# regeirk/pycwt

Hardware: NVIDIA H100
Metric: cwt_scale_points_per_sec (higher is better)
Workload: dtype f64

## Files before the change

### profiles/micro/coarse_ab.py

```python
import os
import subprocess
import sys

import numpy as np

ROOT = os.path.dirname(os.path.dirname(os.path.dirname(os.path.abspath(__file__))))
sys.path.insert(0, ROOT)
import workloads as wl
import pycwt_b200 as pycwt
from pycwt_b200 import _engine
from pycwt_b200.wavelet import _boxcar_len
from bench import pin_to_gpu_numa_node


def identical(arms, fn):
    a, b = (fn(e) for e in arms.values())
    if isinstance(a, tuple):
        return all(np.array_equal(x, y) for x, y in zip(a, b) if x is not None)
    return np.array_equal(a, b)


def main():
    args = sys.argv[1:]
    parent = args[0]
    new = args[1] if len(args) > 1 and not args[1].isdigit() else os.path.join(ROOT, "pycwt_b200", "libcwtb200.so")
    rounds = int(args[-1]) if args[-1].isdigit() else 6
    pin_to_gpu_numa_node(0)
    print(subprocess.run(["nvidia-smi", "--query-gpu=name,power.limit,clocks.max.sm", "--format=csv"],
                         capture_output=True, text=True).stdout.strip())
    c = wl.C2
    x = wl.config2_signal()
    sj = wl.config2_scales()
    arms = {"parent": _engine.Engine(0, lib_path=parent), "new": _engine.Engine(0, lib_path=new)}
    dev = {}
    launches = {}
    for name, eng in arms.items():
        d = eng.dev_alloc(x.nbytes)
        eng.h2d(d, x)
        eng.cwt_dev(d, 0, c["n"], c["dt"], sj, _engine.MORLET, c["f0"], _engine.F64)
        eng.bench_last(10)
        launches[name] = eng.last_launch_count()
        dev[name] = d
    times = {k: [] for k in arms}
    for _ in range(rounds):
        for name, eng in arms.items():
            times[name].append(eng.bench_last(20))
    for name, t in times.items():
        print("%-6s config 2 step %.4f ms (min %.4f, max %.4f) over %d runs of 20 steps, %d launches per step" % (
            name, float(np.median(t)), min(t), max(t), len(t), launches[name]))
    print("median difference parent - new: %.4f ms" % (float(np.median(times["parent"])) - float(np.median(times["new"]))))
    for name, eng in arms.items():
        print(name + ": serialised kernels of one step")
        for k in sorted(eng.profile_last(), key=lambda k: -k["ms"]):
            print("      %-52s %3d x  %7.4f ms  rows %d" % (k["name"], k["launches"], k["ms"], k["rows"]))
    same = True
    for r0 in range(0, len(sj), 32):

        rows = []
        for eng in arms.values():
            out = np.empty((32, c["n"]), np.complex128)
            eng._check(eng.lib.cwtb_get_w(eng.h, _engine._ptr(out), 1, r0, 32))
            rows.append(out)
        same = same and np.array_equal(rows[0], rows[1])
    print("config 2 W (fp64, 256 rows): %s" % ("bit-identical" if same else "DIFFERENT"))
    for name, eng in arms.items():
        eng.dev_free(dev[name])
    c3 = wl.C3
    x3 = wl.config3_signal()
    for fam, code in (("dog", _engine.DOG), ("paul", _engine.PAUL)):
        p = c3[fam]
        s3 = wl.geometric_scales(p["s0"], p["dj"], p["J"])
        for name, eng in arms.items():
            d = eng.dev_alloc(x3.nbytes)
            eng.h2d(d, x3)
            eng.cwt_dev(d, 1, c3["n"], c3["dt"], s3, code, float(p["m"]), _engine.F32)
            eng.bench_last(10)
            launches[name] = eng.last_launch_count()
            dev[name] = d
        times = {k: [] for k in arms}
        for _ in range(rounds):
            for name, eng in arms.items():
                times[name].append(eng.bench_last(20))
        for name, t in times.items():
            print("%-6s config 3 %-4s step %.4f ms (min %.4f, max %.4f), %d launches per step" % (
                name, fam, float(np.median(t)), min(t), max(t), launches[name]))
        for name, eng in arms.items():
            print("%s: serialised kernels of one config 3 %s step" % (name, fam))
            for k in sorted(eng.profile_last(), key=lambda k: -k["ms"]):
                print("      %-52s %3d x  %7.4f ms  rows %d" % (k["name"], k["launches"], k["ms"], k["rows"]))
            eng.dev_free(dev[name])
    print("config 3 Paul(4) W (fp32): %s" % ("bit-identical" if identical(
        arms, lambda e: e.cwt(x3, c3["dt"], s3, _engine.PAUL, float(p["m"]), _engine.F32)) else "DIFFERENT"))
    c4 = wl.C4
    y1, y2 = wl.config4_signals()
    s4 = wl.geometric_scales(c4["s0"], c4["dj"], c4["J"])
    klen = _boxcar_len(pycwt.Morlet(c4["f0"]), c4["dj"])
    for prec, pname in ((_engine.F64, "fp64"), (_engine.F32, "fp32")):
        ok_x = identical(arms, lambda e: e.xwt(y1, y2, c4["dt"], s4, _engine.MORLET, c4["f0"], prec))
        ok_w = identical(arms, lambda e: e.wct(y1, y2, c4["dt"], c4["dj"], s4, _engine.MORLET, c4["f0"], klen,
                                               True, prec))
        print("config 4 %s: xwt %s, wct %s" % (pname, "bit-identical" if ok_x else "DIFFERENT",
                                               "bit-identical" if ok_w else "DIFFERENT"))
    for eng in arms.values():
        eng.close()


if __name__ == "__main__":
    main()
```

### pycwt_b200/csrc/engine.cu

```cuda
#include <algorithm>
#include <array>
#include <cmath>
#include <cstdint>
#include <cstdio>
#include <cstdlib>
#include <cstring>
#include <map>
#include <mutex>
#include <set>
#include <string>
#include <type_traits>
#include <vector>

#include <cuda_runtime.h>
#ifndef CWTB_HOST_EMU
#include <dlfcn.h>
#endif

#include "../../include/cwt_b200.h"
#include "kernels.cuh"

using namespace cwtb;

template <class B, class = void> struct BodyNT { static constexpr int value = NT; };
// ... 92 lines not shown
  int log2N = 0;
  int S = 0;
  int nbatch = 1;
  double dt = 0;
  Fam fam{};
  std::vector<ScaleDesc> descs;
  std::vector<ClassRun> classes;
  std::vector<int> plan_log2K;
  std::vector<double> scales;
  size_t b_single = 0;
  size_t coarse_elems = 0;
  int sig_is_f32 = 0;
  bool exact = false;
  std::vector<OsGroup> os_groups;
};

struct BluePlan {
  unsigned n = 0, L = 0;
  double2 *wm = nullptr;
  double2 *bf[2] = {nullptr, nullptr};
};

struct NTabDev {
  double2 *hi = nullptr, *lo = nullptr;
  int h = 0;
};

struct cwtb_ctx {
  int device = 0;
  rt_stream stream{};
  rt_stream aux_stream{};
  rt_stream prio_stream{};
  rt_stream prio_short{};
  int prio_mode = 1;
  rt_stream chain_streams[3]{};
  int n_chains = 2;
  rt_stream cur{};
  int pad_pow2 = 1;
  int coh_precision = 0;
  std::map<unsigned, BluePlan> blue;
  long long serial = 0;
  int two_streams = 1;
  int three_streams = 1;
  rt_stream copy_streams[4]{};
  int d2h_split = 1;
  std::string err;
  double band_eps = 1e-16;
  double band_eps32 = 1e-9;
  double expand_eps = 5e-13;
  double expand_eps32 = 2e-7;
  int expand_mma = 1;
  int dense_margin = 2;
  int expand_min_log2R = 0;
  int os_on = 1;
  Buf osH, osgrp;
  void *comm = nullptr;
  int comm_world = 1, comm_rank = 0;
  Buf comm_send, comm_recv;
  int group = 0;
  size_t group_bytes = (size_t)512 << 20;
  size_t rows_chunk_bytes = (size_t)256 << 20;
  int l2_persist = 0;
  int direct_max_log2 = 13;
  int fused = 0;
  int ring = 3;
  int pipe_ahead = 2;
  int num_sms = 132;
// ... 749 lines not shown
}

template <typename T> struct FusedArgs {
  PassAArgs<T> a;
  PassBArgs<T> b;
  unsigned *ctr;
  int nscales, ring;
  unsigned tilesA, tilesB;
};

HD void fused_decode(unsigned t, int n, unsigned TA, unsigned TB, int *isB, int *s, unsigned *tile) {
  if (t < TA) { *isB = 0; *s = 0; *tile = t; return; }
  t -= TA;
  const unsigned per = TA + TB;
  const unsigned blk = t / per, off = t % per;
  if ((int)blk < n - 1) {
    if (off < TA) { *isB = 0; *s = (int)blk + 1; *tile = off; }
    else { *isB = 1; *s = (int)blk; *tile = off - TA; }
  } else {
    *isB = 1; *s = n - 1; *tile = t - (unsigned)(n - 1) * per;
  }
}

#ifndef CWTB_HOST_EMU
__device__ __forceinline__ unsigned ld_acquire_u32(const unsigned *p) {
  unsigned v;
  asm volatile("ld.acquire.gpu.global.u32 %0, [%1];" : "=r"(v) : "l"(p) : "memory");
  return v;
}
template <typename T, int K1, int MODE>
__global__ void __launch_bounds__(TileCfg<T>::NT, 3) k_fused(const __grid_constant__ FusedArgs<T> f) {
  extern __shared__ __align__(16) unsigned char smraw[];
  __shared__ unsigned s_t;
  using A = PassABody<T, K1, MODE, +1>;
  using B = PassBBody<T, +1>;
  const int n = f.nscales;
  const unsigned total = (unsigned)n * (f.tilesA + f.tilesB);
  unsigned *doneA = f.ctr + 1, *doneB = f.ctr + 1 + n;
  for (;;) {
    __syncthreads();
    if (threadIdx.x == 0) s_t = atomicAdd(f.ctr, 1u);
    __syncthreads();
    const unsigned t = s_t;
    if (t >= total) break;
    int isB, s;
    unsigned tile;
    fused_decode(t, n, f.tilesA, f.tilesB, &isB, &s, &tile);
    if (threadIdx.x == 0) {
      if (isB) {
        while (ld_acquire_u32(&doneA[s]) < f.tilesA) __nanosleep(100);
      } else if (s >= f.ring) {
        while (ld_acquire_u32(&doneB[s - f.ring]) < f.tilesB) __nanosleep(100);
      }
      asm volatile("fence.proxy.async;" ::: "memory");
    }
    __syncthreads();
    if (isB) run_phases_at<B, 0>(f.b, (int)tile, s, smraw);
    else run_phases_at<A, 0>(f.a, (int)tile, s, smraw);
    __syncthreads();
    if (threadIdx.x == 0)
      asm volatile("red.release.gpu.global.add.u32 [%0], %1;" ::"l"(isB ? &doneB[s] : &doneA[s]), "r"(1u) : "memory");
  }
}
#endif

template <typename T, int K1, int MODE>
static int launch_fused(cwtb_ctx *c, const PassAArgs<T> &a, const PassBArgs<T> &b, int nscales) {
  using A = PassABody<T, K1, MODE, +1>;
  using B = PassBBody<T, +1>;
  FusedArgs<T> f;
  f.a = a; f.b = b;
  f.nscales = nscales;
  f.ring = c->ring;
  f.a.zmod = f.b.zmod = c->ring;
  const unsigned M = a.N / ((unsigned)K1 * K2C);
  f.tilesA = M * (K2C / A::T2);
  f.tilesB = (a.N / K2C + Lay<T, K2C>::P - 1) / Lay<T, K2C>::P;
  int e = ensure(c, c->ctr, (size_t)(1 + 2 * nscales) * sizeof(unsigned));
  if (e) return e;
  f.ctr = (unsigned *)c->ctr.p;
  RT(rt_memset(c->ctr.p, 0, (size_t)(1 + 2 * nscales) * sizeof(unsigned), c->stream));
#ifdef CWTB_HOST_EMU
  std::vector<unsigned char> sm(std::max(A::SMEM, B::SMEM) + 64);
  const unsigned total = (unsigned)nscales * (f.tilesA + f.tilesB);
  for (unsigned t = 0; t < total; ++t) {
    int isB, s;
    unsigned tile;
    fused_decode(t, nscales, f.tilesA, f.tilesB, &isB, &s, &tile);
    if (isB) emu_phases<B, 0>(f.b, (int)tile, s, sm.data());
    else emu_phases<A, 0>(f.a, (int)tile, s, sm.data());
  }
  c->launches++;
  return 0;
#else
  const size_t smem = std::max(A::SMEM, B::SMEM);
  auto kern = k_fused<T, K1, MODE>;
  const void *fn = (const void *)kern;
  if (!c->configured.count(fn)) {
    RT(cudaFuncSetAttribute(kern, cudaFuncAttributeMaxDynamicSharedMemorySize, (int)smem));
    c->configured.insert(fn);
  }
// ... 36 lines not shown
    case 10: return launch_fused<T, 1024, MODE>(c, a, b, n);
  }
  return fail(c, CWTB_ERR_UNSUPPORTED, "transform longer than 2^20 per row is not supported yet");
}

template <typename T> struct PipeArgs {
  PassAArgs<T> a;
  PassBArgs<T> b;
  unsigned *ctr;
  int nscales, ring, ahead;
  unsigned tilesA, tilesB;
};

HD void pipe_decode(unsigned t, int n, int ahead, unsigned TA, unsigned TB, int *isB, int *s, unsigned *tile) {
  const int na = ahead < n ? ahead : n;
  if (t < (unsigned)na * TA) { *isB = 0; *s = (int)(t / TA); *tile = t % TA; return; }
  t -= (unsigned)na * TA;
  const unsigned per = TA + TB;
  const int nmid = n - na;
  if (t < (unsigned)nmid * per) {
    const unsigned blk = t / per, off = t % per;
    if (off < TA) { *isB = 0; *s = na + (int)blk; *tile = off; }
    else { *isB = 1; *s = (int)blk; *tile = off - TA; }
    return;
  }
  t -= (unsigned)nmid * per;
  *isB = 1; *s = nmid + (int)(t / TB); *tile = t % TB;
}

#ifndef CWTB_HOST_EMU
template <typename T, int K1, int MODE>
__global__ void __launch_bounds__(TileCfg<T>::NT, 3) k_pipe(const __grid_constant__ PipeArgs<T> f) {
  extern __shared__ __align__(16) unsigned char smraw[];
  using A = PassABody<T, K1, MODE, +1>;
  using B = PassBBody<T, +1>;
  const int n = f.nscales;
  const unsigned total = (unsigned)n * (f.tilesA + f.tilesB);
  unsigned *doneA = f.ctr, *doneB = f.ctr + n;
  int okA = -1, okB = -1;
  for (unsigned t = blockIdx.x; t < total; t += gridDim.x) {
    int isB, s;
    unsigned tile;
    pipe_decode(t, n, f.ahead, f.tilesA, f.tilesB, &isB, &s, &tile);
    const int dep = isB ? s : s - f.ring;
    if (dep >= 0 && dep > (isB ? okA : okB)) {
      if (threadIdx.x == 0) {
        const unsigned *flag = isB ? &doneA[dep] : &doneB[dep];
        const unsigned want = isB ? f.tilesA : f.tilesB;
        while (ld_acquire_u32(flag) < want) __nanosleep(64);
        asm volatile("fence.proxy.async;" ::: "memory");
      }
      __syncthreads();
      if (isB) okA = dep; else okB = dep;
    }
    if (isB) run_phases_at<B, 0>(f.b, (int)tile, s, smraw);
    else run_phases_at<A, 0>(f.a, (int)tile, s, smraw);
    __syncthreads();
    if (threadIdx.x == blockDim.x - 1) {
      asm volatile("red.release.gpu.global.add.u32 [%0], %1;" ::"l"(isB ? &doneB[s] : &doneA[s]), "r"(1u) : "memory");
    }
  }
}
#endif

template <typename T, int K1, int MODE>
static int launch_pipe(cwtb_ctx *c, const PassAArgs<T> &a, const PassBArgs<T> &b, int nscales) {
  using A = PassABody<T, K1, MODE, +1>;
  using B = PassBBody<T, +1>;
  PipeArgs<T> f;
  f.a = a; f.b = b;
  f.nscales = nscales;
  f.ring = c->ring;
  f.ahead = std::max(1, std::min(c->pipe_ahead, c->ring - 1));
  f.a.zmod = f.b.zmod = c->ring;
  f.b.rev = 0; f.b.pf_dist = 0; f.a.pf_dist = 0;
  const unsigned M = a.N / ((unsigned)K1 * K2C);
  f.tilesA = M * (K2C / A::T2);
  f.tilesB = (a.N / K2C + Lay<T, K2C>::P - 1) / Lay<T, K2C>::P;
  int e = ensure(c, c->ctr, (size_t)(2 * nscales) * sizeof(unsigned));
  if (e) return e;
  f.ctr = (unsigned *)c->ctr.p;
  RT(rt_memset(c->ctr.p, 0, (size_t)(2 * nscales) * sizeof(unsigned), c->cur));
#ifdef CWTB_HOST_EMU
  std::vector<unsigned char> sm(std::max(A::SMEM, B::SMEM) + 64);
  const unsigned total = (unsigned)nscales * (f.tilesA + f.tilesB);
  std::vector<int> seenA(nscales, 0), seenB(nscales, 0);
  for (unsigned t = 0; t < total; ++t) {
    int isB, s;
    unsigned tile;
    pipe_decode(t, nscales, f.ahead, f.tilesA, f.tilesB, &isB, &s, &tile);
    if (isB && seenA[s] != (int)f.tilesA) return fail(c, CWTB_ERR_STATE, "pipe schedule: B before its A tiles");
    if (!isB && s >= f.ring && seenB[s - f.ring] != (int)f.tilesB)
      return fail(c, CWTB_ERR_STATE, "pipe schedule: Z slot reused before its B tiles");
    if (isB) { emu_phases<B, 0>(f.b, (int)tile, s, sm.data()); seenB[s]++; }
    else { emu_phases<A, 0>(f.a, (int)tile, s, sm.data()); seenA[s]++; }
  }
  c->launches++;
  return 0;
#else
  const size_t smem = std::max(A::SMEM, B::SMEM);
// ... 674 lines not shown
int cwtb_host_free(cwtb_ctx *c, void *p) {
  if (!c || !c->pinned.count(p)) return CWTB_ERR_ARG;
  c->pinned.erase(p);
  rt_host_free(p);
  return 0;
}
int cwtb_dev_alloc(cwtb_ctx *c, size_t bytes, void **out) {
  if (!c || !out) return CWTB_ERR_ARG;
  if (rt_malloc(out, bytes) != 0) return fail(c, CWTB_ERR_NOMEM, "device allocation failed");
  c->devallocs.insert(*out);
  return 0;
}
int cwtb_dev_free(cwtb_ctx *c, void *p) {
  if (!c || !c->devallocs.count(p)) return CWTB_ERR_ARG;
  c->devallocs.erase(p);
  rt_free(p);
  return 0;
}
int cwtb_memcpy_h2d(cwtb_ctx *c, void *dst, const void *src, size_t bytes) {
  RT(rt_h2d(dst, src, bytes, c->stream));
  RT(rt_sync(c->stream));
  return 0;
}
int cwtb_memcpy_d2h(cwtb_ctx *c, void *dst, const void *src, size_t bytes) {
  RT(rt_d2h(dst, src, bytes, c->stream));
  RT(rt_sync(c->stream));
  return 0;
}
int cwtb_sync(cwtb_ctx *c) {
  RT(rt_sync(c->stream));
  return 0;
}

static const double kOsUs = 9.5;
static const double kTwoKernelUs = 23.2;

struct DevTmp {
  void *p = nullptr;
  ~DevTmp() { if (p) rt_free(p); }
};

static int os_plan(cwtb_ctx *c, const Job &job, double dt, int family, double param, std::vector<OsRow> &os) {
  constexpr int L = OsBody<4>::L, GR = 4;
  auto os_cheaper = [](int M) { return M <= L / 2 && kOsUs * L / (double)(L - M + 1) < kTwoKernelUs; };
  os.assign(job.S, OsRow());
  const unsigned N = job.N;
  if (!c->os_on || job.precision != CWTB_F64 || job.exact || family == CWTB_TABLE ||
      !(c->band_eps > 0) || !(c->expand_eps > 0) || N < 2u * L)
    return 0;
  const long long half = (long long)N / 2;
  std::vector<int> cand;
  std::vector<double> cs;
  for (const ScaleDesc &d : job.descs) {
    if (d.chan != 0 || d.k_hi < d.k_lo || d.k_lo <= -half || d.k_hi >= ((long long)N - 1) / 2) continue;
    if (d.ip_log2Nc || (d.log2K <= 10 || (d.log2K <= c->direct_max_log2 && d.log2K < job.log2N))) continue;
    cand.push_back(d.row);
    cs.push_back(d.s);
  }
  if (cand.empty()) return 0;
  const int nc = (int)cand.size();
  const size_t wcap = (size_t)job.S * job.nbatch * job.n0;
  const int chunk = (int)std::max<size_t>(1, wcap / N);
  int e = ensure(c, c->W, std::max<size_t>((size_t)chunk * N, wcap) * sizeof(double2));
  if (e) return e;
  double2 *h = (double2 *)c->W.p;
  DevTmp dimp, part;
  if (rt_malloc(&dimp.p, (size_t)N * sizeof(double))) return fail(c, CWTB_ERR_NOMEM, "device allocation failed");
  {
// ... 1546 lines not shown
```

### pycwt_b200/csrc/fft_tile.cuh

```cuda
#pragma once
#include "cplx.cuh"

namespace cwtb {

#ifndef CWTB_NT
#define CWTB_NT 128
#endif
#ifndef CWTB_NT_F32
#define CWTB_NT_F32 256
#endif
#ifndef CWTB_TILE_F64
#define CWTB_TILE_F64 4096
#endif
#ifndef CWTB_TILE_F32
#define CWTB_TILE_F32 8192
#endif
#ifndef CWTB_MINB
#define CWTB_MINB 1
#endif
#ifndef CWTB_UNROLL_B
#define CWTB_UNROLL_B 1
#endif
#define CWTB_STR_(x) #x
#define CWTB_STR(x) CWTB_STR_(x)
#define CWTB_PRAGMA_UNROLL_B _Pragma(CWTB_STR(unroll CWTB_UNROLL_B))
#ifndef CWTB_PASSA_BATCH
#define CWTB_PASSA_BATCH 8
#endif
#ifndef CWTB_UNROLL_A
#define CWTB_UNROLL_A 4
#endif
#define CWTB_PRAGMA_UNROLL_A _Pragma(CWTB_STR(unroll CWTB_UNROLL_A))
constexpr int NT = CWTB_NT;
#ifndef CWTB_PLAN1024_R32
#define CWTB_PLAN1024_R32 0
#endif
#ifndef CWTB_PLAN256_3PASS
#define CWTB_PLAN256_3PASS 1
#endif
HD constexpr int tw_radix(int L) {
  return L == 32 ? 4 : (L == 256 ? (CWTB_PLAN256_3PASS ? 4 : 16) : ((L == 1024 && CWTB_PLAN1024_R32) ? 32 : 8));
}
// ... 210 lines not shown
    V e = nroot_t<T>(nt, (unsigned)base * pk2);
    const V se = nroot_t<T>(nt, (unsigned)stride * pk2);
    const V ne = nroot_t<T>(nt, (unsigned)(-K) * pk2);
#pragma unroll
    for (int i = 0; i < R; ++i) {
      tw[i] = (base + i * stride >= rsplit_row) ? cmul(e, ne) : e;
      e = cmul(e, se);
    }
  }
  HD void load(int b, V (&x)[R]) const {
#pragma unroll
    for (int i = 0; i < R; ++i) x[i] = cmul(sm[Lay<T, K>::phys(b, base + i * stride)], tw[i]);
  }
};

template <typename T, int K> struct RowLoader {
  using V = cx<T>;
  const V *src;
  int nvalid;
  int base, stride;
  HD void begin(int base_, int stride_, int, int) { base = base_; stride = stride_; }
  template <int R> HD void load(int b, V (&x)[R]) const {
    if (b < nvalid) {
      const V *row = src + (size_t)b * K + base;
#pragma unroll
      for (int i = 0; i < R; ++i) x[i] = row[i * stride];
    } else {
#pragma unroll
      for (int i = 0; i < R; ++i) x[i] = mk<T>(0, 0);
    }
  }
};

template <typename T, int K, int R> struct GenLoader {
  using V = cx<T>;
  static constexpr int P = Lay<T, K>::P;
  static constexpr int I = K / R;
  static constexpr int NT = TileCfg<T>::NT;
  static constexpr int GROUPS = (I >= NT) ? 1 : NT / I;
  static constexpr bool ONE_SHOT = (P / GROUPS <= 1);
  const V *B;
  NTab nt;
  int rsplit;
  unsigned p0;
  V a[ONE_SHOT ? 1 : R], d[ONE_SHOT ? 1 : R];
  int base, stride;
  unsigned pp;
  HD void begin(int base_, int stride_, int bstart, int bstep) {
    base = base_; stride = stride_;
    pp = p0 + (unsigned)bstart;
    if (ONE_SHOT) return;
    V e = nroot_t<T>(nt, (unsigned)base * pp);
    V de = nroot_t<T>(nt, (unsigned)base * (unsigned)bstep);
    const V se = nroot_t<T>(nt, (unsigned)stride * pp);
    const V sd = nroot_t<T>(nt, (unsigned)stride * (unsigned)bstep);
    const V ne = nroot_t<T>(nt, (unsigned)(-K) * pp);
    const V nd = nroot_t<T>(nt, (unsigned)(-K) * (unsigned)bstep);
#pragma unroll
    for (int i = 0; i < R; ++i) {
      const int r = base + i * stride;
      const bool neg = r >= rsplit;
      d[ONE_SHOT ? 0 : i] = neg ? cmul(de, nd) : de;
      a[ONE_SHOT ? 0 : i] = cmul(ldg(&B[r]), neg ? cmul(e, ne) : e);
      e = cmul(e, se);
      de = cmul(de, sd);
    }
  }
  HD void load(int, V (&x)[R]) {
    if (ONE_SHOT) {
      V e = nroot_t<T>(nt, (unsigned)base * pp);
      const V se = nroot_t<T>(nt, (unsigned)stride * pp);
      const V ne = nroot_t<T>(nt, (unsigned)(-K) * pp);
#pragma unroll
      for (int i = 0; i < R; ++i) {
        const int r = base + i * stride;
        x[i] = cmul(ldg(&B[r]), (r >= rsplit) ? cmul(e, ne) : e);
        e = cmul(e, se);
      }
      return;
    }
#pragma unroll
    for (int i = 0; i < R; ++i) { x[i] = a[ONE_SHOT ? 0 : i]; a[ONE_SHOT ? 0 : i] = cmul(a[ONE_SHOT ? 0 : i], d[ONE_SHOT ? 0 : i]); }
  }
};

template <typename T, int K, int L, int R, int SIGN, class Loader, bool ROWS = false>
HD void pass_mid(cx<T> *sm, const cx<T> *__restrict__ tw, Loader &ld, int tid) {
  using V = cx<T>;
  using LY = Lay<T, K, ROWS>;
  constexpr int NT = TileCfg<T>::NT;
  constexpr int Ln = L / R, I = K / R, P = LY::P;
  constexpr int LANES = (I >= NT) ? NT : I;
  constexpr int GROUPS = NT / LANES;
  const int tp0 = tid % LANES, bg = tid / LANES;
  for (int tp = tp0; tp < I; tp += LANES) {
    const int g = tp / Ln, j = tp % Ln;
    V twv[R];
#pragma unroll
    static_assert(tw_radix(L) == R, "pass twiddle table was built for another radix");
    for (int c = 1; c < R; ++c) {
      V w = ldg(&tw[tw_offset(L) + (c - 1) * Ln + j]);
      if (SIGN < 0) w.y = -w.y;
      twv[c] = w;
    }
    ld.begin(g * L + j, Ln, bg, GROUPS);
    CWTB_PRAGMA_UNROLL_B
    for (int b = bg; b < P; b += GROUPS) {
      V x[R];
      ld.load(b, x);
      dftR<R, SIGN, T>(x);
#pragma unroll
      for (int c = 1; c < R; ++c) x[c] = cmul(x[c], twv[c]);
#pragma unroll
      for (int c = 0; c < R; ++c) sm[LY::phys(b, g * L + c * Ln + j)] = x[c];
    }
  }
}

template <typename T, int K, int SIGN, class Storer, bool ROWS = false, bool GMAJOR = false>
HD void pass_last(const cx<T> *sm, Storer &st, int tid) {
  using V = cx<T>;
  using LY = Lay<T, K, ROWS>;
  constexpr int NT = TileCfg<T>::NT;
  constexpr int R = Plan<K>::RL, G = K / R, P = LY::P;
  for (int idx = tid; idx < G * P; idx += NT) {
    const int b = GMAJOR ? idx / G : idx % P, g = GMAJOR ? idx % G : idx / P;
    V x[R];
#pragma unroll
    for (int i = 0; i < R; ++i) x[i] = sm[LY::phys(b, g * R + i)];
    dftR<R, SIGN, T>(x);
    st.store(b, Plan<K>::qlow(g), G, x);
  }
}

template <typename T, int K> struct TilePhases {
  static constexpr int NP = Plan<K>::NP;
};

template <typename T, int K, int SIGN, class Loader, bool ROWS = false>
HD void tile_first(cx<T> *sm, const cx<T> *tw, Loader &ld, int tid) {
  pass_mid<T, K, K, Plan<K>::R1, SIGN, Loader, ROWS>(sm, tw, ld, tid);
}
template <typename T, int K, int SIGN, bool ROWS = false>
HD void tile_second(cx<T> *sm, const cx<T> *tw, int tid) {
  SmemLoader<T, K, ROWS> ld;
  ld.sm = sm;
  pass_mid<T, K, K / Plan<K>::R1, Plan<K>::R2, SIGN, SmemLoader<T, K, ROWS>, ROWS>(sm, tw, ld, tid);
}

}
```

### pycwt_b200/csrc/kernels.cuh

```cuda
#pragma once
#include <math.h>
#include "fft_tile.cuh"

namespace cwtb {

struct ScaleDesc {
  double s;
  double amp;
  int row;
  int k_lo, k_hi;
  int log2K;
  int rsplit;
  int trow;
  int chan;
  int pad_;
  long long boff;
  int ip_log2Nc;
  int ip_kc;
  int ip_w;
  int os_grp;
  long long ip_coff;
  long long ip_woff;
  double ip_beta;
  double ip_dc;
// ... 402 lines not shown
      st.U = U;
      st.ostride = il;
      st.ooff = (a.by0 + by) % il;
      st.epi.mode = a.epi;
      if (a.epi == EPI_GAUSS) {
        st.epi.g = a.grow[row];
        st.epi.invn = 1.0 / ((double)a.N * il);
        st.epi.post = a.post;
        st.epi.nfreq = (long long)a.N * il;
      }
      pass_last<T, K, SIGN, OutStorer<T>, true>(sm, st, tid);
      if (tid == 0) tb.inval();
    }
  }
};

struct OsGroup {
  int first, count;
  int t1, hop;
  long long hoff;
};
struct OsArgs {
  const ScaleDesc *descs;
  const OsGroup *groups;
  const double *sig;
  const double2 *H;
  double2 *W;
  const double2 *tw;
  long long n0;
  unsigned N;
  int epi;
};

template <int L, int R> struct OsSigLoader {
  const double *x;
  long long start, n0;
  unsigned nmask;
  int hop, base, stride;
  HD void begin(int base_, int stride_, int, int) { base = base_; stride = stride_; }
  HD void load(int b, double2 (&v)[R]) const {
    const long long s = start + (long long)b * hop + base;
#pragma unroll
    for (int i = 0; i < R; ++i) {
      const long long n = (s + (long long)i * stride) & (long long)nmask;
      v[i] = make_double2(n < n0 ? ldg(&x[n]) : 0.0, 0.0);
    }
  }
};
template <int L> struct OsHalfStorer {
  double2 *xs;
  template <int R> HD void store(int b, int ql, int qs, double2 (&x)[R]) const {
#pragma unroll
    for (int c = 0; c < R; ++c) {
      const int q = ql + c * qs;
      if (q <= L / 2) xs[b * (L / 2 + 1) + q] = x[c];
    }
  }
};
template <int L, int R> struct OsSpecLoader {
  const double2 *xs, *H;
  int base, stride;
  double2 hv[R];
  HD void begin(int base_, int stride_, int, int) {
    base = base_; stride = stride_;
#pragma unroll
    for (int i = 0; i < R; ++i) hv[i] = ldg(&H[base + i * stride]);
  }
  HD void load(int b, double2 (&v)[R]) const {
#pragma unroll
    for (int i = 0; i < R; ++i) {
      const int q = base + i * stride;
      const double2 y = q <= L / 2 ? xs[b * (L / 2 + 1) + q] : cconj(xs[b * (L / 2 + 1) + L - q]);
      v[i] = cmul(y, hv[i]);
    }
  }
};
struct OsStorer {
  double2 *row;
  long long nb0, n0;
  int t1, hop, epi;
  template <int R> HD void store(int b, int ql, int qs, double2 (&x)[R]) const {
    const long long nb = nb0 + (long long)b * hop;
#pragma unroll
    for (int c = 0; c < R; ++c) {
      const int i = ql + c * qs;
      const long long n = nb + i;
      if (i >= t1 && i < t1 + hop && n < n0) {
        if (epi == EPI_STORE) st_stream(&row[n], x[c]);
        else row[n] = cmul(row[n], cconj(x[c]));
      }
    }
  }
};

template <int G> struct OsBody {
  static constexpr int L = 1024;
  static constexpr int NTB = TileCfg<double>::NT;
  static constexpr int NT = NTB;
  using Args = OsArgs;
  using LY = Lay<double, L>;
  static constexpr int P = LY::P;
  static_assert(Plan<L>::NP == 3, "overlap-save phases assume a three-pass tile plan");
  static constexpr int NPHASE = 3 + 3 * G;
  static constexpr size_t SMEM = LY::TILE_BYTES + (size_t)P * (L / 2 + 1) * sizeof(double2);
  template <int PH> HD static void phase(const Args &a, int bx, int by, int tid, void *smraw) {
    double2 *sm = (double2 *)smraw;
    double2 *xs = (double2 *)((char *)smraw + LY::TILE_BYTES);
    const OsGroup g = a.groups[by];
    const long long n_first = (long long)bx * P * g.hop;
    if (n_first >= a.n0) return;
    if constexpr (PH == 0) {
      OsSigLoader<L, Plan<L>::R1> ld;
      ld.x = a.sig + (size_t)a.descs[g.first].chan * a.n0; ld.start = n_first - g.t1; ld.n0 = a.n0; ld.nmask = a.N - 1; ld.hop = g.hop;
      tile_first<double, L, -1>(sm, a.tw, ld, tid);
    } else if constexpr (PH == 1) {
      tile_second<double, L, -1>(sm, a.tw, tid);
    } else if constexpr (PH == 2) {
      OsHalfStorer<L> st{xs};
      pass_last<double, L, -1, OsHalfStorer<L>, false, true>(sm, st, tid);
    } else {
      constexpr int r = (PH - 3) / 3, step = (PH - 3) % 3;
      if (r >= g.count) return;
      if constexpr (step == 0) {
        OsSpecLoader<L, Plan<L>::R1> ld;
        ld.xs = xs; ld.H = a.H + g.hoff + (long long)r * L;
        tile_first<double, L, +1>(sm, a.tw, ld, tid);
      } else if constexpr (step == 1) {
        tile_second<double, L, +1>(sm, a.tw, tid);
      } else {
        OsStorer st;
        st.row = a.W + (size_t)a.descs[g.first + r].row * a.n0;
        st.nb0 = n_first - g.t1; st.n0 = a.n0; st.t1 = g.t1; st.hop = g.hop; st.epi = a.epi;
        pass_last<double, L, +1, OsStorer, false, true>(sm, st, tid);
      }
    }
  }
};

struct AbsMaxArgs { const double2 *h; double *out; long long pitch, lo, hi; int nblk; };
struct AbsMaxBody {
  using Args = AbsMaxArgs;
  static constexpr int NPHASE = 2;
  static constexpr size_t SMEM = NT * sizeof(double);
  template <int PH> HD static void phase(const Args &a, int bx, int by, int tid, void *smraw) {
    double *sm = (double *)smraw;
    if constexpr (PH == 0) {
      const long long chunk = (a.hi - a.lo + a.nblk - 1) / a.nblk;
      const long long s = a.lo + bx * chunk, e = s + chunk < a.hi ? s + chunk : a.hi;
      double m = 0;
      for (long long i = s + tid; i < e; i += NT) {
        const double2 v = a.h[(size_t)by * a.pitch + i];
        m = fmax(m, fmax(fabs(v.x), fabs(v.y)));
      }
      sm[tid] = m;
    } else if (tid == 0) {
      double m = 0;
      for (int i = 0; i < NT; ++i) m = fmax(m, sm[i]);
      a.out[(size_t)by * a.nblk + bx] = m;
    }
  }
};

enum { MODE_DENSE = 0, MODE_BAND = 1, MODE_REAL = 2, MODE_CPLX = 3, MODE_COARSE = 4 };

template <typename T> HD cx<T> coarse_value(const Fam &fam, const ScaleDesc &d, const cx<T> *spec, int r, unsigned Nx) {
  const int Nc = 1 << d.ip_log2Nc;
  const int kp = r < Nc / 2 ? r : r - Nc;
  const int k = d.ip_kc + kp;
  if (k < d.k_lo || k > d.k_hi) return mk<T>(0, 0);
  const cx<T> b = band_value<T>(fam, d, spec, (unsigned)k & (Nx - 1), k, Nx);
  const double pw = 3.14159265358979323846 * (double)d.ip_w;
  const double x = pw * ((double)kp / (double)Nc);
  const double bb = d.ip_beta * d.ip_beta;
  const double z = sqrt(fma(-x, x, bb));
  const double f = d.ip_dc * (z / sinh(z));
  return mk<T>((T)((double)b.x * f), (T)((double)b.y * f));
}

template <typename T> struct PassAArgs {
  const ScaleDesc *descs;
  const cx<T> *spec;
  const cx<T> *Bbuf;
  const void *in;
  cx<T> *Z;
  const cx<T> *tw;
  Fam fam;
  NTab nt;
  long long in_pitch, n_in;
  unsigned N;
  int first, row0;
  int zmod;
  int pf_dist;
  int gauss_rec;
  unsigned K2;
  unsigned Nx;
};

template <typename T, int K1, int MODE, int SIGN> struct PassABody {
  static constexpr int NTB = TileCfg<T>::NT;
  static constexpr int NT = NTB;
  using V = cx<T>;
  using Args = PassAArgs<T>;
  using LY = Lay<T, K1>;
  static constexpr int NP = Plan<K1>::NP;
  static constexpr int P = LY::P;
  static constexpr int T2 = P < K2C ? P : K2C;
  static constexpr int NPHASE = NP == 1 ? 1 : NP + 1;
  static constexpr size_t SMEM = LY::BYTES;

  struct Src {
    const Args &a;
    ScaleDesc d;
    int by, p;
    V twist0;
    HD Src(const Args &a_, int by_, int p_) : a(a_), by(by_), p(p_) {
      if (MODE == MODE_DENSE || MODE == MODE_BAND || MODE == MODE_COARSE) d = a.descs[a.first + by];
    }
    HD V get(int pos, int r2) const {
      const unsigned r = (unsigned)pos * a.K2 + (unsigned)r2;
      if (MODE == MODE_DENSE) {
        const int k = (int)r - (r >= a.N / 2 ? (int)a.N : 0);
        if (a.fam.family != 3 && (k < d.k_lo || k > d.k_hi)) return mk<T>(0, 0);
        return band_value<T>(a.fam, d, a.spec, r, k, a.N);
      } else if (MODE == MODE_BAND) {
        V v = ldg(&a.Bbuf[d.boff + r]);
        if (p == 0 || NP > 1) return v;
        const int k1 = pos - ((int)r >= d.rsplit ? K1 : 0);
        V w = nroot_t<T>(a.nt, (unsigned)k1 * (unsigned)p * a.K2);
        return cmul(v, w);
      } else if (MODE == MODE_COARSE) {
        return coarse_value<T>(a.fam, d, a.spec, (int)r, a.Nx);
      } else if (MODE == MODE_REAL) {
        const T *row = (const T *)a.in + (size_t)(a.row0 + by) * a.in_pitch;
// ... 95 lines not shown
              kprev = k;
              v = cscale(raw[u], (T)(g * d.amp));
            } else {
              since = 1 << 30;
            }
            sm[LY::phys(b, pos)] = v;
          }
        }
      } else if (CWTB_PASSA_ASYNC && MODE == MODE_BAND) {
        const V *base = a.Bbuf + src.d.boff + r20;
        for (int idx = tid; idx < K1 * T2; idx += NT) {
          const int b = idx % T2, pos = idx / T2;
          cp_async(&sm[LY::phys(b, pos)], base + (size_t)pos * a.K2 + b);
        }
        cp_async_wait();
      } else if (CWTB_PASSA_ASYNC && MODE == MODE_CPLX) {
        const V *row = (const V *)a.in + (size_t)(a.row0 + by) * a.in_pitch;
        for (int idx = tid; idx < K1 * T2; idx += NT) {
          const int b = idx % T2, pos = idx / T2;
          const unsigned r = (unsigned)pos * a.K2 + (unsigned)(r20 + b);
          if ((long long)r < a.n_in) cp_async(&sm[LY::phys(b, pos)], row + r);
          else sm[LY::phys(b, pos)] = mk<T>(0, 0);
        }
        cp_async_wait();
      } else {
        CWTB_PRAGMA_UNROLL_A
        for (int idx = tid; idx < K1 * T2; idx += NT) {
          const int b = idx % T2, pos = idx / T2;
          sm[LY::phys(b, pos)] = src.get(pos, r20 + b);
        }
      }
    } else if constexpr (PH == 1) {
      if (MODE == MODE_BAND && p != 0) {
        SmemTwistLoader<T, K1, Plan<K1>::R1> ld;
        ld.sm = sm;
        ld.nt = a.nt;
        ld.rsplit_row = a.descs[a.first + by].rsplit / (int)a.K2;
        ld.pk2 = (unsigned)p * a.K2;
        tile_first<T, K1, SIGN>(sm, a.tw, ld, tid);
      } else {
        SmemLoader<T, K1> ld;
        ld.sm = sm;
        tile_first<T, K1, SIGN>(sm, a.tw, ld, tid);
      }
    } else if constexpr (PH == 2 && NP == 3) {
      tile_second<T, K1, SIGN>(sm, a.tw, tid);
    } else {
      pass_last<T, K1, SIGN>(sm, st, tid);
    }
  }
};

struct CoarseSeg { int first, count, log2Nc, cta0; };
constexpr int CSEG_MAX = 32;
HD constexpr size_t cmax(size_t a, size_t b) { return a > b ? a : b; }
template <typename T> struct CoarseArgs {
  const ScaleDesc *descs;
  const cx<T> *spec;
  cx<T> *Z;
  cx<T> *C;
  const cx<T> *tw;
  Fam fam;
  NTab nt[11];
  unsigned Nx;
  int nseg;
  int pf_dist, rev;
  CoarseSeg seg[CSEG_MAX];
};
template <typename T> HD const CoarseSeg &coarse_seg(const CoarseArgs<T> &a, int bx) {
  int s = 0;
  while (s + 1 < a.nseg && bx >= a.seg[s + 1].cta0) ++s;
  return a.seg[s];
}

template <typename T> struct CoarseRowsBody {
  static constexpr int NTB = TileCfg<T>::NT;
  static constexpr int NT = NTB;
  using V = cx<T>;
  using Args = CoarseArgs<T>;
  template <int K> static constexpr size_t bytes() { return Lay<T, K>::BYTES; }
  static constexpr size_t SMEM = cmax(cmax(cmax(bytes<64>(), bytes<128>()), cmax(bytes<256>(), bytes<512>())), bytes<1024>());
// ... 1319 lines not shown
```

Before: 110.5 billion.

## Pair overlap-save forward FFTs as complex, shrink thread counts, retune plan costs

The overlap-save kernel now packs two real signal blocks into one complex FFT, as real and imaginary parts, and separates their half spectra in a new phase. This halves the forward transform work per tile. Thread counts for the overlap-save and fp64 dense pass-A bodies become separately configurable (default 128), and the templates are threaded with NT and block-count parameters. The stream priority mode default and the planner's cost constants are also changed. Results can differ from the previous version at rounding level, and the A/B script now reports per-row relative differences instead of requiring bit-identity.

```diff
diff --git a/profiles/micro/coarse_ab.py b/profiles/micro/coarse_ab.py
--- a/profiles/micro/coarse_ab.py
+++ b/profiles/micro/coarse_ab.py
@@ -13,11 +13,31 @@
 from bench import pin_to_gpu_numa_node
 
 
-def identical(arms, fn):
+def row_diff(a, b):
+    a = np.atleast_2d(a)
+    b = np.atleast_2d(b)
+    both = np.isnan(a) & np.isnan(b)
+    d = np.where(both, 0, np.abs(a - b)).max(axis=1)
+    m = np.where(both, 0, np.abs(a)).max(axis=1)
+    return np.where(m > 0, d / np.where(m > 0, m, 1), d)
+
+
+def max_row_diff(arms, fn):
     a, b = (fn(e) for e in arms.values())
-    if isinstance(a, tuple):
-        return all(np.array_equal(x, y) for x, y in zip(a, b) if x is not None)
-    return np.array_equal(a, b)
+    pairs = zip(a, b) if isinstance(a, tuple) else [(a, b)]
+    return max(float(row_diff(x, y).max()) for x, y in pairs if x is not None)
+
+
+def describe(d):
+    return "bit-identical" if d == 0 else "max per-row difference %.2e" % d
+
+
+def plan_class(code, log2n):
+    if code == -2:
+        return "overlap-save"
+    if code < -2:
+        return "expansion"
+    return "dense" if code == log2n else "exact"
 
 
 def main():
@@ -53,16 +73,24 @@
         print(name + ": serialised kernels of one step")
         for k in sorted(eng.profile_last(), key=lambda k: -k["ms"]):
             print("      %-52s %3d x  %7.4f ms  rows %d" % (k["name"], k["launches"], k["ms"], k["rows"]))
-    same = True
+    plans = {name: eng.last_plan(len(sj)) for name, eng in arms.items()}
+    log2n = int(np.log2(arms["new"].padded_length()))
+    diff = np.empty(len(sj))
     for r0 in range(0, len(sj), 32):
-
         rows = []
         for eng in arms.values():
             out = np.empty((32, c["n"]), np.complex128)
             eng._check(eng.lib.cwtb_get_w(eng.h, _engine._ptr(out), 1, r0, 32))
             rows.append(out)
-        same = same and np.array_equal(rows[0], rows[1])
-    print("config 2 W (fp64, 256 rows): %s" % ("bit-identical" if same else "DIFFERENT"))
+        diff[r0:r0 + 32] = row_diff(rows[0], rows[1])
+    if plans["parent"] != plans["new"]:
+        print("config 2: the arms plan different row classes")
+    cls = np.array([plan_class(p, log2n) for p in plans["new"]])
+    for k in ("overlap-save", "dense", "exact", "expansion"):
+        sel = cls == k
+        if sel.any():
+            print("config 2 W (fp64) %-12s rows %3d: max per-row difference %.2e of the row's maximum, "
+                  "%d rows not bit-identical" % (k, sel.sum(), diff[sel].max(), int((diff[sel] != 0).sum())))
     for name, eng in arms.items():
         eng.dev_free(dev[name])
     c3 = wl.C3
@@ -89,18 +117,17 @@
             for k in sorted(eng.profile_last(), key=lambda k: -k["ms"]):
                 print("      %-52s %3d x  %7.4f ms  rows %d" % (k["name"], k["launches"], k["ms"], k["rows"]))
             eng.dev_free(dev[name])
-    print("config 3 Paul(4) W (fp32): %s" % ("bit-identical" if identical(
-        arms, lambda e: e.cwt(x3, c3["dt"], s3, _engine.PAUL, float(p["m"]), _engine.F32)) else "DIFFERENT"))
+    print("config 3 Paul(4) W (fp32): %s" % describe(max_row_diff(
+        arms, lambda e: e.cwt(x3, c3["dt"], s3, _engine.PAUL, float(p["m"]), _engine.F32))))
     c4 = wl.C4
     y1, y2 = wl.config4_signals()
     s4 = wl.geometric_scales(c4["s0"], c4["dj"], c4["J"])
     klen = _boxcar_len(pycwt.Morlet(c4["f0"]), c4["dj"])
     for prec, pname in ((_engine.F64, "fp64"), (_engine.F32, "fp32")):
-        ok_x = identical(arms, lambda e: e.xwt(y1, y2, c4["dt"], s4, _engine.MORLET, c4["f0"], prec))
-        ok_w = identical(arms, lambda e: e.wct(y1, y2, c4["dt"], c4["dj"], s4, _engine.MORLET, c4["f0"], klen,
-                                               True, prec))
-        print("config 4 %s: xwt %s, wct %s" % (pname, "bit-identical" if ok_x else "DIFFERENT",
-                                               "bit-identical" if ok_w else "DIFFERENT"))
+        d_x = max_row_diff(arms, lambda e: e.xwt(y1, y2, c4["dt"], s4, _engine.MORLET, c4["f0"], prec))
+        d_w = max_row_diff(arms, lambda e: e.wct(y1, y2, c4["dt"], c4["dj"], s4, _engine.MORLET, c4["f0"], klen,
+                                                 True, prec))
+        print("config 4 %s: xwt %s, wct %s" % (pname, describe(d_x), describe(d_w)))
     for eng in arms.values():
         eng.close()
 
diff --git a/pycwt_b200/csrc/engine.cu b/pycwt_b200/csrc/engine.cu
--- a/pycwt_b200/csrc/engine.cu
+++ b/pycwt_b200/csrc/engine.cu
@@ -148,7 +148,7 @@
   rt_stream aux_stream{};
   rt_stream prio_stream{};
   rt_stream prio_short{};
-  int prio_mode = 1;
+  int prio_mode = 2;
   rt_stream chain_streams[3]{};
   int n_chains = 2;
   rt_stream cur{};
@@ -964,7 +964,7 @@
 __global__ void __launch_bounds__(TileCfg<T>::NT, 3) k_fused(const __grid_constant__ FusedArgs<T> f) {
   extern __shared__ __align__(16) unsigned char smraw[];
   __shared__ unsigned s_t;
-  using A = PassABody<T, K1, MODE, +1>;
+  using A = PassABody<T, K1, MODE, +1, TileCfg<T>::NT>;
   using B = PassBBody<T, +1>;
   const int n = f.nscales;
   const unsigned total = (unsigned)n * (f.tilesA + f.tilesB);
@@ -998,7 +998,7 @@
 
 template <typename T, int K1, int MODE>
 static int launch_fused(cwtb_ctx *c, const PassAArgs<T> &a, const PassBArgs<T> &b, int nscales) {
-  using A = PassABody<T, K1, MODE, +1>;
+  using A = PassABody<T, K1, MODE, +1, TileCfg<T>::NT>;
   using B = PassBBody<T, +1>;
   FusedArgs<T> f;
   f.a = a; f.b = b;
@@ -1101,7 +1101,7 @@
 template <typename T, int K1, int MODE>
 __global__ void __launch_bounds__(TileCfg<T>::NT, 3) k_pipe(const __grid_constant__ PipeArgs<T> f) {
   extern __shared__ __align__(16) unsigned char smraw[];
-  using A = PassABody<T, K1, MODE, +1>;
+  using A = PassABody<T, K1, MODE, +1, TileCfg<T>::NT>;
   using B = PassBBody<T, +1>;
   const int n = f.nscales;
   const unsigned total = (unsigned)n * (f.tilesA + f.tilesB);
@@ -1134,7 +1134,7 @@
 
 template <typename T, int K1, int MODE>
 static int launch_pipe(cwtb_ctx *c, const PassAArgs<T> &a, const PassBArgs<T> &b, int nscales) {
-  using A = PassABody<T, K1, MODE, +1>;
+  using A = PassABody<T, K1, MODE, +1, TileCfg<T>::NT>;
   using B = PassBBody<T, +1>;
   PipeArgs<T> f;
   f.a = a; f.b = b;
@@ -1875,8 +1875,8 @@
   return 0;
 }
 
-static const double kOsUs = 9.5;
-static const double kTwoKernelUs = 23.2;
+static const double kOsUs = 9.1;
+static const double kTwoKernelUs = 23.6;
 
 struct DevTmp {
   void *p = nullptr;
diff --git a/pycwt_b200/csrc/fft_tile.cuh b/pycwt_b200/csrc/fft_tile.cuh
--- a/pycwt_b200/csrc/fft_tile.cuh
+++ b/pycwt_b200/csrc/fft_tile.cuh
@@ -8,6 +8,12 @@
 #endif
 #ifndef CWTB_NT_F32
 #define CWTB_NT_F32 256
+#endif
+#ifndef CWTB_NT_OS
+#define CWTB_NT_OS 128
+#endif
+#ifndef CWTB_NT_DENSE
+#define CWTB_NT_DENSE 128
 #endif
 #ifndef CWTB_TILE_F64
 #define CWTB_TILE_F64 4096
@@ -284,11 +290,10 @@
   }
 };
 
-template <typename T, int K, int R> struct GenLoader {
+template <typename T, int K, int R, int NT = TileCfg<T>::NT> struct GenLoader {
   using V = cx<T>;
   static constexpr int P = Lay<T, K>::P;
   static constexpr int I = K / R;
-  static constexpr int NT = TileCfg<T>::NT;
   static constexpr int GROUPS = (I >= NT) ? 1 : NT / I;
   static constexpr bool ONE_SHOT = (P / GROUPS <= 1);
   const V *B;
@@ -336,12 +341,12 @@
   }
 };
 
-template <typename T, int K, int L, int R, int SIGN, class Loader, bool ROWS = false>
+template <typename T, int K, int L, int R, int SIGN, class Loader, bool ROWS = false, int NT = TileCfg<T>::NT,
+          int PB = Lay<T, K, ROWS>::P>
 HD void pass_mid(cx<T> *sm, const cx<T> *__restrict__ tw, Loader &ld, int tid) {
   using V = cx<T>;
   using LY = Lay<T, K, ROWS>;
-  constexpr int NT = TileCfg<T>::NT;
-  constexpr int Ln = L / R, I = K / R, P = LY::P;
+  constexpr int Ln = L / R, I = K / R, P = PB;
   constexpr int LANES = (I >= NT) ? NT : I;
   constexpr int GROUPS = NT / LANES;
   const int tp0 = tid % LANES, bg = tid / LANES;
@@ -369,12 +374,12 @@
   }
 }
 
-template <typename T, int K, int SIGN, class Storer, bool ROWS = false, bool GMAJOR = false>
+template <typename T, int K, int SIGN, class Storer, bool ROWS = false, bool GMAJOR = false, int NT = TileCfg<T>::NT,
+          int PB = Lay<T, K, ROWS>::P>
 HD void pass_last(const cx<T> *sm, Storer &st, int tid) {
   using V = cx<T>;
   using LY = Lay<T, K, ROWS>;
-  constexpr int NT = TileCfg<T>::NT;
-  constexpr int R = Plan<K>::RL, G = K / R, P = LY::P;
+  constexpr int R = Plan<K>::RL, G = K / R, P = PB;
   for (int idx = tid; idx < G * P; idx += NT) {
     const int b = GMAJOR ? idx / G : idx % P, g = GMAJOR ? idx % G : idx / P;
     V x[R];
@@ -389,15 +394,16 @@
   static constexpr int NP = Plan<K>::NP;
 };
 
-template <typename T, int K, int SIGN, class Loader, bool ROWS = false>
+template <typename T, int K, int SIGN, class Loader, bool ROWS = false, int NT = TileCfg<T>::NT,
+          int PB = Lay<T, K, ROWS>::P>
 HD void tile_first(cx<T> *sm, const cx<T> *tw, Loader &ld, int tid) {
-  pass_mid<T, K, K, Plan<K>::R1, SIGN, Loader, ROWS>(sm, tw, ld, tid);
-}
-template <typename T, int K, int SIGN, bool ROWS = false>
+  pass_mid<T, K, K, Plan<K>::R1, SIGN, Loader, ROWS, NT, PB>(sm, tw, ld, tid);
+}
+template <typename T, int K, int SIGN, bool ROWS = false, int NT = TileCfg<T>::NT, int PB = Lay<T, K, ROWS>::P>
 HD void tile_second(cx<T> *sm, const cx<T> *tw, int tid) {
   SmemLoader<T, K, ROWS> ld;
   ld.sm = sm;
-  pass_mid<T, K, K / Plan<K>::R1, Plan<K>::R2, SIGN, SmemLoader<T, K, ROWS>, ROWS>(sm, tw, ld, tid);
-}
-
-}
+  pass_mid<T, K, K / Plan<K>::R1, Plan<K>::R2, SIGN, SmemLoader<T, K, ROWS>, ROWS, NT, PB>(sm, tw, ld, tid);
+}
+
+}
diff --git a/pycwt_b200/csrc/kernels.cuh b/pycwt_b200/csrc/kernels.cuh
--- a/pycwt_b200/csrc/kernels.cuh
+++ b/pycwt_b200/csrc/kernels.cuh
@@ -458,29 +458,31 @@
   int epi;
 };
 
-template <int L, int R> struct OsSigLoader {
+template <int L, int R> struct OsPairLoader {
   const double *x;
   long long start, n0;
   unsigned nmask;
-  int hop, base, stride;
+  int hop, nblk, base, stride;
   HD void begin(int base_, int stride_, int, int) { base = base_; stride = stride_; }
+  HD double at(long long n) const {
+    n &= (long long)nmask;
+    return n < n0 ? ldg(&x[n]) : 0.0;
+  }
   HD void load(int b, double2 (&v)[R]) const {
-    const long long s = start + (long long)b * hop + base;
+    const long long s = start + (long long)(2 * b) * hop + base;
+    const bool re = 2 * b < nblk, im = 2 * b + 1 < nblk;
 #pragma unroll
     for (int i = 0; i < R; ++i) {
-      const long long n = (s + (long long)i * stride) & (long long)nmask;
-      v[i] = make_double2(n < n0 ? ldg(&x[n]) : 0.0, 0.0);
-    }
-  }
-};
-template <int L> struct OsHalfStorer {
-  double2 *xs;
+      const long long n = s + (long long)i * stride;
+      v[i] = make_double2(re ? at(n) : 0.0, im ? at(n + hop) : 0.0);
+    }
+  }
+};
+template <int PF> struct OsPairStorer {
+  double2 *sm;
   template <int R> HD void store(int b, int ql, int qs, double2 (&x)[R]) const {
 #pragma unroll
-    for (int c = 0; c < R; ++c) {
-      const int q = ql + c * qs;
-      if (q <= L / 2) xs[b * (L / 2 + 1) + q] = x[c];
-    }
+    for (int c = 0; c < R; ++c) sm[Lay<double, 1024>::phys(PF + b, ql + c * qs)] = x[c];
   }
 };
 template <int L, int R> struct OsSpecLoader {
@@ -521,14 +523,18 @@
 
 template <int G> struct OsBody {
   static constexpr int L = 1024;
-  static constexpr int NTB = TileCfg<double>::NT;
+  static constexpr int NTB = CWTB_NT_OS;
   static constexpr int NT = NTB;
+  static constexpr int MINB = NT > 128 ? 2 : 1;
   using Args = OsArgs;
   using LY = Lay<double, L>;
   static constexpr int P = LY::P;
+  static constexpr int PF = P / 2;
+  static constexpr int H = L / 2 + 1;
   static_assert(Plan<L>::NP == 3, "overlap-save phases assume a three-pass tile plan");
-  static constexpr int NPHASE = 3 + 3 * G;
-  static constexpr size_t SMEM = LY::TILE_BYTES + (size_t)P * (L / 2 + 1) * sizeof(double2);
+  static_assert(P % 2 == 0, "overlap-save blocks are transformed in pairs");
+  static constexpr int NPHASE = 4 + 3 * G;
+  static constexpr size_t SMEM = LY::TILE_BYTES + (size_t)P * H * sizeof(double2);
   template <int PH> HD static void phase(const Args &a, int bx, int by, int tid, void *smraw) {
     double2 *sm = (double2 *)smraw;
     double2 *xs = (double2 *)((char *)smraw + LY::TILE_BYTES);
@@ -536,28 +542,39 @@
     const long long n_first = (long long)bx * P * g.hop;
     if (n_first >= a.n0) return;
     if constexpr (PH == 0) {
-      OsSigLoader<L, Plan<L>::R1> ld;
+      using LD = OsPairLoader<L, Plan<L>::R1>;
+      LD ld;
       ld.x = a.sig + (size_t)a.descs[g.first].chan * a.n0; ld.start = n_first - g.t1; ld.n0 = a.n0; ld.nmask = a.N - 1; ld.hop = g.hop;
-      tile_first<double, L, -1>(sm, a.tw, ld, tid);
+      const long long nb = (a.n0 - n_first + g.hop - 1) / g.hop;
+      ld.nblk = nb < P ? (int)nb : P;
+      tile_first<double, L, -1, LD, false, NT, PF>(sm, a.tw, ld, tid);
     } else if constexpr (PH == 1) {
-      tile_second<double, L, -1>(sm, a.tw, tid);
+      tile_second<double, L, -1, false, NT, PF>(sm, a.tw, tid);
     } else if constexpr (PH == 2) {
-      OsHalfStorer<L> st{xs};
-      pass_last<double, L, -1, OsHalfStorer<L>, false, true>(sm, st, tid);
+      OsPairStorer<PF> st{sm};
+      pass_last<double, L, -1, OsPairStorer<PF>, false, true, NT, PF>(sm, st, tid);
+    } else if constexpr (PH == 3) {
+      for (int idx = tid; idx < PF * H; idx += NT) {
+        const int b = idx / H, k = idx % H;
+        const double2 y = sm[LY::phys(PF + b, k)], z = cconj(sm[LY::phys(PF + b, (L - k) & (L - 1))]);
+        xs[(2 * b) * H + k] = make_double2(0.5 * (y.x + z.x), 0.5 * (y.y + z.y));
+        xs[(2 * b + 1) * H + k] = make_double2(0.5 * (y.y - z.y), -0.5 * (y.x - z.x));
+      }
     } else {
-      constexpr int r = (PH - 3) / 3, step = (PH - 3) % 3;
+      constexpr int r = (PH - 4) / 3, step = (PH - 4) % 3;
       if (r >= g.count) return;
       if constexpr (step == 0) {
-        OsSpecLoader<L, Plan<L>::R1> ld;
+        using LD = OsSpecLoader<L, Plan<L>::R1>;
+        LD ld;
         ld.xs = xs; ld.H = a.H + g.hoff + (long long)r * L;
-        tile_first<double, L, +1>(sm, a.tw, ld, tid);
+        tile_first<double, L, +1, LD, false, NT>(sm, a.tw, ld, tid);
       } else if constexpr (step == 1) {
-        tile_second<double, L, +1>(sm, a.tw, tid);
+        tile_second<double, L, +1, false, NT>(sm, a.tw, tid);
       } else {
         OsStorer st;
         st.row = a.W + (size_t)a.descs[g.first + r].row * a.n0;
         st.nb0 = n_first - g.t1; st.n0 = a.n0; st.t1 = g.t1; st.hop = g.hop; st.epi = a.epi;
-        pass_last<double, L, +1, OsStorer, false, true>(sm, st, tid);
+        pass_last<double, L, +1, OsStorer, false, true, NT>(sm, st, tid);
       }
     }
   }
@@ -622,9 +639,14 @@
   unsigned Nx;
 };
 
-template <typename T, int K1, int MODE, int SIGN> struct PassABody {
-  static constexpr int NTB = TileCfg<T>::NT;
+template <typename T, int MODE> HD constexpr int passa_nt() {
+  return (sizeof(T) == 8 && MODE == MODE_DENSE) ? CWTB_NT_DENSE : TileCfg<T>::NT;
+}
+
+template <typename T, int K1, int MODE, int SIGN, int NTA = passa_nt<T, MODE>()> struct PassABody {
+  static constexpr int NTB = NTA;
   static constexpr int NT = NTB;
+  static constexpr int MINB = NTA > TileCfg<T>::NT ? 2 : CWTB_MINB;
   using V = cx<T>;
   using Args = PassAArgs<T>;
   using LY = Lay<T, K1>;
@@ -786,21 +808,22 @@
       }
     } else if constexpr (PH == 1) {
       if (MODE == MODE_BAND && p != 0) {
-        SmemTwistLoader<T, K1, Plan<K1>::R1> ld;
+        using TL = SmemTwistLoader<T, K1, Plan<K1>::R1>;
+        TL ld;
         ld.sm = sm;
         ld.nt = a.nt;
         ld.rsplit_row = a.descs[a.first + by].rsplit / (int)a.K2;
         ld.pk2 = (unsigned)p * a.K2;
-        tile_first<T, K1, SIGN>(sm, a.tw, ld, tid);
+        tile_first<T, K1, SIGN, TL, false, NT>(sm, a.tw, ld, tid);
       } else {
         SmemLoader<T, K1> ld;
         ld.sm = sm;
-        tile_first<T, K1, SIGN>(sm, a.tw, ld, tid);
+        tile_first<T, K1, SIGN, SmemLoader<T, K1>, false, NT>(sm, a.tw, ld, tid);
       }
     } else if constexpr (PH == 2 && NP == 3) {
-      tile_second<T, K1, SIGN>(sm, a.tw, tid);
+      tile_second<T, K1, SIGN, false, NT>(sm, a.tw, tid);
     } else {
-      pass_last<T, K1, SIGN>(sm, st, tid);
+      pass_last<T, K1, SIGN, ZStorer<T, SIGN>, false, false, NT>(sm, st, tid);
     }
   }
 };
```

New measurement: 112.7 billion (median of 6 runs). 2.0% higher.
